# FindoraNetwork/ark-bulletproofs

Hardware: AMD Instinct MI355X
Metric: r1cs_constraints_proved_per_sec (+ r1cs_batch_verifies_per_sec under "verify") (higher is better)
Workload: dtype u32x9 (256-bit modular integers, radix 2^29)

## Files before the change

### ark_bulletproofs_amd/_lib.py

```python
import ctypes as C
import os

import numpy as np

_HERE = os.path.dirname(os.path.abspath(__file__))
LIB_PATH = os.environ.get("ARKBP_LIB_PATH") or os.path.join(_HERE, "libarkbp_hip.so")
_lib = None

BP_OK, BP_E_ARG, BP_E_HIP, BP_E_NO_DEVICE, BP_E_VERIFICATION, BP_E_GENS_LENGTH, BP_E_FORMAT, BP_E_MISSING = 0, -1, -2, -3, -4, -5, -6, -7

EXPORTS = [
    "bp_last_error", "bp_device_count", "bp_ctx_create", "bp_ctx_destroy", "bp_ctx_sync",
    "bp_dev_alloc", "bp_dev_free", "bp_dev_upload", "bp_dev_download", "bp_points_import", "bp_points_export",
    "bp_msm", "bp_msm_gens", "bp_msm_dev", "bp_msm_window_count", "bp_msm_dev_windows", "bp_ipa_create", "bp_ipa_begin", "bp_ipa_round_LR", "bp_ipa_round_fold", "bp_ipa_finish", "bp_ipa_export", "bp_ipa_verify", "bp_gens_derive", "bp_gens_upload", "bp_gens_download", "bp_pedersen_gens",
    "bp_host_derive_generators", "bp_transcript_new", "bp_transcript_free", "bp_transcript_append_message", "bp_transcript_challenge_bytes",
    "bp_transcript_append_point", "bp_transcript_challenge_scalar", "bp_host_sha3_512", "bp_host_points_sum", "bp_debug_rng_draws", "bp_debug_append_points_x8", "bp_debug_challenge_x8", "bp_r1cs_prove_scenario", "bp_stmt_prover_create", "bp_stmt_free", "bp_stmt_info", "bp_stmt_prove", "bp_stmt_precompute", "bp_stmt_precompute_batch", "bp_gens_share", "bp_r1cs_verification_gh", "bp_r1cs_verify_scenario", "bp_r1cs_batch_verify_scenarios", "bp_ctx_set_profiling", "bp_ctx_kernel_time", "bp_ctx_reset_profiling",
    "bp_debug_decompress", "bp_debug_field_op", "bp_debug_point_op", "bp_debug_glv_decompose", "bp_ctx_set_tuning", "bp_ctx_set_window_shard", "bp_pedersen_commit_batch", "bp_stmt_prover_create_dev",
    "bp_prover_new", "bp_verifier_new", "bp_verifier_new_like", "bp_cs_free", "bp_cs_transcript", "bp_cs_metrics", "bp_prover_commit", "bp_verifier_commit",
    "bp_cs_multiply", "bp_cs_allocate", "bp_cs_allocate_multiplier", "bp_cs_constrain", "bp_cs_allocate_multipliers", "bp_cs_constrain_many",
    "bp_cs_specify_randomized_constraints", "bp_cs_challenge_scalar", "bp_prover_set_rng", "bp_prover_precompute", "bp_prover_precompute_batch", "bp_prover_prove", "bp_prover_prove_batch", "bp_prover_commit_batch", "bp_ctx_prove_batch_stats",
    "bp_ctx_set_shard_allgather", "bp_gens_fold_tables", "bp_gens_msm_tables", "bp_debug_exp_iter", "bp_debug_inner_product", "bp_verifier_verify", "bp_r1cs_batch_verify", "bp_stmt_as_prover", "bp_transcript_export_state", "bp_transcript_import_state", "bp_transcript_clone",
    "bp_gens_tables_check", "bp_debug_tables_ptr", "bp_rccl_unique_id", "bp_ctx_rccl_init", "bp_ctx_rccl_shutdown", "bp_ctx_collective_stats", "bp_debug_rccl_allgather",
    "bp_debug_vfe_schedule_replay", "bp_debug_vfe_schedule_replay_2phase", "bp_debug_vfe_challenges", "bp_ctx_vfe_stats", "bp_debug_verify_challenges", "bp_debug_ctx_create_hostonly", "bp_ctx_msm_stats", "bp_ctx_direct_stats", "bp_gens_direct_tables", "bp_ctx_fold_stats", "bp_gens_fold_tables_slice",
]


class ArkbpError(RuntimeError):
    def __init__(self, code, where):
        self.code = code
        msg = lib().bp_last_error().decode(errors="replace") if _lib is not None else ""
        super().__init__("%s failed with code %d: %s" % (where, code, msg))


def lib():
    global _lib
    if _lib is None:
        if not os.path.exists(LIB_PATH):
            raise ImportError(
# ... 25 lines not shown
```

### ark_bulletproofs_amd/csrc/arkbp.hip

```cpp
#include <hip/hip_runtime.h>
#include <sys/prctl.h>
#include <time.h>
#include <rccl/rccl.h>
#include <dlfcn.h>
#include <mutex>
#include <cmath>
#include <cstdio>
#include <cstring>
#include <algorithm>
#include <array>
#include <functional>
#include <map>
#include <memory>
#include <set>
#include <string>
#include <unordered_map>
#include <vector>
#include "../../include/arkbp.h"
#include <atomic>
#include <chrono>
#include "host_proto.hpp"
#include "r1cs.cuh"
#include "pedersen.cuh"
#include "small.cuh"
// ... 153 lines not shown
    bool have_gf = false, have_rho = false;
    F4 gf_halves[2];
    const F4* rho_pw = nullptr;
    const u32* d_rho_pow = nullptr;
    bool lr_done = false;
    bool allow_freeze = false, frozen = false;
    size_t n0 = 0;
    u32 *d_cG = nullptr, *d_cH = nullptr;
    u32 gens_first = 0, gens_stride = 0;
    const u32 *d_G_in = nullptr, *d_H_in = nullptr;
    bool have_qw = false;
    F4 qw;
    int msm_mode = -1;
    bool deferred = false;
    F4 def_tG, def_tH;
    size_t min_len = 0;
    bool direct = false;
    bool fold_pending = false;
    F4 pend_u, pend_ui;
    u32 *d_a_alt = nullptr, *d_b_alt = nullptr;
    F4 geo_k0;
    bool have_k0 = false;
};

struct bp_ctx {
    int curve = 0, device = 0;
    bool host_only = false;
    hipStream_t stream = nullptr;
    bool profiling = false;
    size_t tune_fold_batch_min = 65536;
// ... 49 lines not shown
    void* gather_user = nullptr;
    ncclComm_t nccl = nullptr;
    DevBuf coll_send, coll_recv;
    void* h_coll = nullptr;
    size_t h_coll_cap = 0;
    uint64_t coll_count = 0;
    double coll_seconds = 0;
    size_t tune_cyclic_min = (size_t)1 << 14;
    size_t tune_msm_fixed_min = (size_t)1 << 20;
    size_t tune_host_threads = 0;
    hipEvent_t sync_ev_aux = nullptr;
    unsigned tune_wait_sleep = 0;
    bool msm_latency_first = false;
    size_t tune_msm_chunk_cap = 0;
    size_t tune_fold_quad_max = 0;
    size_t tune_msm_glv_min = 256;
    DevBuf cyc_a, cyc_b, cyc_Gf, cyc_Hf;
    DevBuf fb_G, fb_H, fb_pc;
    size_t fb_cap = 0;
    DevBuf ftab_G, ftab_H;
    size_t ftab_n = 0;
    u32 ftab_first = 0, ftab_stride = 1;
    int ftab_w = 0, ftab_nwin = 0;
    DevBuf dt_tab, dt_part, dt_a2, dt_b2, dt_ticket;
    size_t dt_cap = 0;
    size_t tune_direct_max = 8192;
    u32* h_dt = nullptr;
    u32 dt_pending_parts = 1;
    uint64_t dt_runs = 0;
    size_t tune_prove_batch = 0;
// ... 989 lines not shown
    if constexpr (C::HAS_GLV) {
        Naf2 g, h;
        if (glv_pair<C>(tG, tH, g, h)) {
            if (quad) hipLaunchKernelGGL((k_ipa_fold_glv<C, true>), dim3(grid), dim3(256), 0, st, d_G, d_H, (u32)n, g, h, which, ff.jac);
            else hipLaunchKernelGGL((k_ipa_fold_glv<C, false>), dim3(grid), dim3(256), 0, st, d_G, d_H, (u32)n, g, h, which, ff.jac);
            done = true;
        }
    }
    if (!done) {
        Naf a = naf_of<S>(tG), b = naf_of<S>(tH);
        if (quad) hipLaunchKernelGGL((k_ipa_fold_uniform<C, true>), dim3(grid), dim3(256), 0, st, d_G, d_H, (u32)n, a, b, which, ff.jac);
        else hipLaunchKernelGGL((k_ipa_fold_uniform<C, false>), dim3(grid), dim3(256), 0, st, d_G, d_H, (u32)n, a, b, which, ff.jac);
    }
    }
    fold_finish_launch<C>(ctx, ff, d_G, d_H, n, which, lanes);
    return BP_OK;
}

static void ftab_recode(const uint64_t* mag, int nl, bool negate, int w, int nwin, unsigned short* e, unsigned long long& negmask) {
    uint64_t k[5] = {0, 0, 0, 0, 0};
    for (int i = 0; i < nl; i++) k[i] = mag[i];
    const uint64_t full = (uint64_t)1 << w, half = full >> 1;
    negmask = 0;
    for (int j = 0; j < nwin; j++) {
        uint64_t d = k[0] & (full - 1);
        for (int i = 0; i < 4; i++) k[i] = (k[i] >> w) | (k[i + 1] << (64 - w));
        k[4] >>= w;
        bool neg = false;
        if (d > half) { d = full - d; neg = true; for (int i = 0; i < 5; i++) if (++k[i]) break; }
        e[j] = (unsigned short)d;
        if (d && (neg != negate)) negmask |= 1ull << j;
// ... 297 lines not shown
            s.lr_done = true;
            return BP_OK;
        }
        BaseSegs sg; memset(&sg, 0, sizeof sg);
        sg.nseg = 3; sg.start[0] = 0; sg.start[1] = (u32)n0; sg.start[2] = (u32)(2 * n0); sg.start[3] = (u32)(2 * n0 + 1);
        sg.ptr[0] = s.d_G; sg.ptr[1] = s.d_H; sg.ptr[2] = s.d_Q;
        J4 Lj, Rj;
        BPCHK(msm_run<C>(ctx, sg, sL, 2 * n0 + 1, 0, Lj, 0, -1, s.msm_mode));
        BPCHK(msm_run<C>(ctx, sg, sR, 2 * n0 + 1, 0, Rj, 0, -1, s.msm_mode));
        A4 La = G::to_aff(Lj), Ra = G::to_aff(Rj);
        memcpy(Lw, La.x.v, 32); memcpy(Lw + 4, La.y.v, 32);
        memcpy(Rw, Ra.x.v, 32); memcpy(Rw + 4, Ra.y.v, 32);
        s.lr_done = true;
        return BP_OK;
    }
    if (s.deferred) {
        const size_t n1 = s.n;
        {
            ScopedK tk(ctx, BP_K_IPA_SCALARS);
            hipLaunchKernelGGL(k_ipa_scalars_deferred<C>, dim3(gb), dim3(256), 0, st, s.d_a, s.d_b, (u32)n, sL, sR, ctx->ipa_part.as<u32>(), s.pending ? (s.h_geo ? 2 : 1) : 0,
                               words_of<S>(s.gamma_G), words_of<S>(s.gamma_H), s.d_rho_pow, words_of<S>(s.def_tG), words_of<S>(s.def_tH));
            hipLaunchKernelGGL(k_ipa_ip_finish<C>, dim3(1), dim3(256), 0, st, ctx->ipa_part.as<u32>(), gb, sL + 4 * n * 8, sR + 4 * n * 8, words_of<S>(s.qw), s.have_qw ? 1 : 0);
        }
        J4 Lj, Rj; bool dl = false, dr = false;
        if (s.msm_mode == 2) {
            BaseSegs sg; memset(&sg, 0, sizeof sg);
            sg.nseg = 5;
            for (int k = 0; k <= 4; k++) sg.start[k] = (u32)(k * n);
            sg.start[5] = (u32)(4 * n + 1);
            const size_t f0 = s.gens_first, sd = s.gens_stride;
            const bool rows = s.have_qw && ctx->fb_cap;
            ScalSegs ss; memset(&ss, 0, sizeof ss);
            ss.nseg = 2; ss.ptr[0] = sL; ss.start[0] = 0; ss.start[1] = (u32)(4 * n); ss.ptr[1] = sL + (4 * n + 1) * 8; ss.start[2] = (u32)(4 * n + 1);
            if (rows) {
                FbRun rl[5] = {{0, f0 + (n1 + n) * sd, n, sd}, {0, f0 + n * sd, n, sd}, {1, f0 + n1 * sd, n, sd}, {1, f0, n, sd}, {2, 0, 1}};
                BPCHK(msm_fixed_run<C>(ctx, rl, 5, ss, 4 * n + 1, 0, Lj, dl, 2));
// ... 5 lines not shown
            if (rows) {
                ss.ptr[0] = sR; ss.ptr[1] = sR + (4 * n + 1) * 8;
                FbRun rr[5] = {{0, f0 + n1 * sd, n, sd}, {0, f0, n, sd}, {1, f0 + (n1 + n) * sd, n, sd}, {1, f0 + n * sd, n, sd}, {2, 0, 1}};
                BPCHK(msm_fixed_run<C>(ctx, rr, 5, ss, 4 * n + 1, 0, Rj, dr, 2));
            }
            if (!dr) {
                sg.ptr[0] = s.d_G_in + n1 * 16; sg.ptr[1] = s.d_G_in; sg.ptr[2] = s.d_H_in + (n1 + n) * 16; sg.ptr[3] = s.d_H_in + n * 16; sg.ptr[4] = s.d_Q;
                BPCHK(msm_run<C>(ctx, sg, sR, 4 * n + 1, 0, Rj, 0, -1, 2));
            }
            A4 La = G::to_aff(Lj), Ra = G::to_aff(Rj);
            memcpy(Lw, La.x.v, 32); memcpy(Lw + 4, La.y.v, 32);
            memcpy(Rw, Ra.x.v, 32); memcpy(Rw + 4, Ra.y.v, 32);
            s.lr_done = true;
            return BP_OK;
        }
        const size_t gofs = (size_t)(s.d_G_in - ctx->d_G.as<u32>()) / 16, hofs = (size_t)(s.d_H_in - ctx->d_H.as<u32>()) / 16;
        if (s.have_qw && s.msm_mode == -1) {
            ScalSegs ss; memset(&ss, 0, sizeof ss);
            ss.nseg = 2; ss.ptr[0] = sL; ss.start[0] = 0; ss.start[1] = (u32)(4 * n); ss.ptr[1] = sL + (4 * n + 1) * 8; ss.start[2] = (u32)(4 * n + 1);
            FbRun rl[5] = {{0, gofs + n1 + n, n}, {0, gofs + n, n}, {1, hofs + n1, n}, {1, hofs, n}, {2, 0, 1}};
            BPCHK(msm_fixed_run<C>(ctx, rl, 5, ss, 4 * n + 1, 0, Lj, dl));
            if (dl) {
                ss.ptr[0] = sR; ss.ptr[1] = sR + (4 * n + 1) * 8;
                FbRun rr[5] = {{0, gofs + n1, n}, {0, gofs, n}, {1, hofs + n1 + n, n}, {1, hofs + n, n}, {2, 0, 1}};
                BPCHK(msm_fixed_run<C>(ctx, rr, 5, ss, 4 * n + 1, 0, Rj, dr));
            }
        }
        if (!(dl && dr)) {
            BaseSegs sg; memset(&sg, 0, sizeof sg);
            sg.nseg = 5;
            for (int k = 0; k <= 4; k++) sg.start[k] = (u32)(k * n);
            sg.start[5] = (u32)(4 * n + 1);
            sg.ptr[0] = s.d_G_in + (n1 + n) * 16; sg.ptr[1] = s.d_G_in + n * 16; sg.ptr[2] = s.d_H_in + n1 * 16; sg.ptr[3] = s.d_H_in; sg.ptr[4] = s.d_Q;
            BPCHK(msm_run<C>(ctx, sg, sL, 4 * n + 1, 0, Lj, 0, -1, s.msm_mode));
            sg.ptr[0] = s.d_G_in + n1 * 16; sg.ptr[1] = s.d_G_in; sg.ptr[2] = s.d_H_in + (n1 + n) * 16; sg.ptr[3] = s.d_H_in + n * 16;
            BPCHK(msm_run<C>(ctx, sg, sR, 4 * n + 1, 0, Rj, 0, -1, s.msm_mode));
        }
        A4 La = G::to_aff(Lj), Ra = G::to_aff(Rj);
        memcpy(Lw, La.x.v, 32); memcpy(Lw + 4, La.y.v, 32);
        memcpy(Rw, Ra.x.v, 32); memcpy(Rw + 4, Ra.y.v, 32);
        s.lr_done = true;
        return BP_OK;
    }
    {
        ScopedK tk(ctx, BP_K_IPA_SCALARS);
        hipLaunchKernelGGL(k_ipa_scalars<C>, dim3(gb), dim3(256), 0, st, s.d_a, s.d_b, s.d_Gf, s.d_Hf, s.first ? 1 : 0, (u32)n, sL, sR, ctx->ipa_part.as<u32>(),
                           s.pending ? (s.h_geo ? 2 : 1) : 0, words_of<S>(s.gamma_G), words_of<S>(s.gamma_H), s.d_rho_pow);
        hipLaunchKernelGGL(k_ipa_ip_finish<C>, dim3(1), dim3(256), 0, st, ctx->ipa_part.as<u32>(), gb, sL + 2 * n * 8, sR + 2 * n * 8, words_of<S>(s.qw), s.have_qw ? 1 : 0);
    }
    if (s.d_G_in && s.have_qw && s.msm_mode == -1) {
// ... 133 lines not shown
                BPCHK(launch_tab_fold2<C>(ctx, s, d_G, d_H, n, t2G, t2H, done2));
                if (done2) ctx->folds_tab2++;
                if (!done2) {
                    bool done1 = false;
                    BPCHK(launch_tab_fold<C>(ctx, s, d_G, d_H, 2 * n, s.def_tG, s.def_tH, done1));
                    if (!done1) {
                        if (s.d_G_in != d_G) {
                        HIPCHK(hipMemcpyAsync(d_G, s.d_G_in, 4 * n * 64, hipMemcpyDeviceToDevice, st));
                        HIPCHK(hipMemcpyAsync(d_H, s.d_H_in, 4 * n * 64, hipMemcpyDeviceToDevice, st));
                        }
                        BPCHK(launch_uniform_fold<C>(ctx, d_G, d_H, 2 * n, s.def_tG, s.def_tH, 3));
                    }
                    BPCHK(launch_uniform_fold<C>(ctx, d_G, d_H, n, t2G, t2H, 3));
                }
                s.deferred = false;
            } else
            BPCHK(launch_uniform_fold<C>(ctx, d_G, d_H, n, S::sqr(ui), s.h_geo ? S::mul(S::sqr(u), s.rho_pw[k]) : S::sqr(u), 3));
            s.gamma_G = S::mul(s.gamma_G, u);
            s.gamma_H = s.h_geo ? S::mul(S::mul(s.gamma_H, ui), s.rho_pw[32 + k]) : S::mul(s.gamma_H, ui);
            s.pending = true;
        }
    }
    HIPCHK(hipGetLastError());
    s.first = false;
    if (!s.deferred) s.d_G_in = s.d_H_in = nullptr;
    s.round++;
    s.n = n;
    s.lr_done = false;
    if (s.allow_freeze && n >= 2 && n <= ctx->tune_ipa_freeze_len) {
        BPCHK(ctx->ipa_cG.ensure(n * 32)); BPCHK(ctx->ipa_cH.ensure(n * 32));
        s.d_cG = ctx->ipa_cG.as<u32>(); s.d_cH = ctx->ipa_cH.as<u32>();
        hipLaunchKernelGGL(k_ipa_freeze_init<C>, dim3((u32)((n + 255) / 256)), dim3(256), 0, st, s.d_cG, s.d_cH, (u32)n, s.pending ? (s.h_geo ? 2 : 1) : 0,
// ... 209 lines not shown
    ctx->ipa_step_active = false;
    if (n == 0 || (n & (n - 1))) { g_err = "ipa_begin: n must be a power of two (reference asserts, src/inner_product_proof.rs:66)"; return BP_E_ARG; }
    BPCHK(ipa_upload_host<C>(ctx, Q, Gf, Hf, Gv, Hv, a, b, n));
    BPCHK(ipa_begin_dev<C>(ctx, ctx->ipa_step, ctx->ipa_Q.as<u32>(), ctx->ipa_Gf.as<u32>(), ctx->ipa_Hf.as<u32>(), ctx->ipa_G.as<u32>(), ctx->ipa_H.as<u32>(),
                           ctx->ipa_a.as<u32>(), ctx->ipa_b.as<u32>(), n, nullptr, nullptr, nullptr));
    ctx->ipa_step_active = true;
    return BP_OK;
}
template <class C>
static int ipa_export_host(bp_ctx* ctx, uint64_t* a, uint64_t* b, uint64_t* G_xy, uint64_t* H_xy, uint64_t gG[4], uint64_t gH[4], size_t* n_cur) {
    typedef typename C::Fr Fr;
    IpaState& s = ctx->ipa_step;
    if (s.lr_done) { g_err = "ipa_export: between round_LR and round_fold"; return BP_E_ARG; }
    hipStream_t st = ctx->stream;
    const size_t n = s.n;
    const u32 gb = (u32)((n + 255) / 256);
    BPCHK(ctx->io_out.ensure(n * 64 * 2 + n * 32 * 2));
    u32* o = ctx->io_out.as<u32>();
    hipLaunchKernelGGL(k_points_dev_to_ark<C>, dim3(gb), dim3(256), 0, st, s.d_G, o, (u32)n);
    hipLaunchKernelGGL(k_points_dev_to_ark<C>, dim3(gb), dim3(256), 0, st, s.d_H, o + n * 16, (u32)n);
    hipLaunchKernelGGL(k_scalars_export<Fr>, dim3(gb), dim3(256), 0, st, s.d_a, o + n * 32, (u32)n);
    hipLaunchKernelGGL(k_scalars_export<Fr>, dim3(gb), dim3(256), 0, st, s.d_b, o + n * 40, (u32)n);
    HIPCHK(hipGetLastError());
    HIPCHK(hipMemcpyAsync(G_xy, o, n * 64, hipMemcpyDeviceToHost, st));
    HIPCHK(hipMemcpyAsync(H_xy, o + n * 16, n * 64, hipMemcpyDeviceToHost, st));
    HIPCHK(hipMemcpyAsync(a, o + n * 32, n * 32, hipMemcpyDeviceToHost, st));
    HIPCHK(hipMemcpyAsync(b, o + n * 40, n * 32, hipMemcpyDeviceToHost, st));
    HIPCHK(ctx_stream_wait(ctx));
    memcpy(gG, s.gamma_G.v, 32); memcpy(gH, s.gamma_H.v, 32);
    *n_cur = n;
// ... 582 lines not shown
    c->gather_cb = cb; c->gather_user = user;
    return BP_OK;
}
int bp_ctx_set_tuning(bp_ctx* c, int knob, uint64_t value) {
    if (!c) return BP_E_ARG;
    switch (knob) {
        case BP_TUNE_CYCLIC_MIN: c->tune_cyclic_min = (size_t)value; return BP_OK;
        case BP_TUNE_MSM_FIXED_MIN: c->tune_msm_fixed_min = (size_t)value; return BP_OK;
        case BP_TUNE_HOST_THREADS: if (value > 256) return BP_E_ARG; c->tune_host_threads = (size_t)value; c->pool.reset(); return BP_OK;
        case BP_TUNE_FOLD_BATCH_MIN: c->tune_fold_batch_min = (size_t)value; return BP_OK;
        case BP_TUNE_MSM_BIN_MIN: c->tune_msm_bin_min = (size_t)value; return BP_OK;
        case BP_TUNE_IPA_FREEZE_LEN: c->tune_ipa_freeze_len = (size_t)value; return BP_OK;
        case BP_TUNE_MSM_WSUM_MIN: c->tune_msm_wsum_min = (size_t)value; return BP_OK;
        case BP_TUNE_MSM_GLV_MIN: c->tune_msm_glv_min = (size_t)value; return BP_OK;
        case BP_TUNE_FOLD_QUAD_MAX: c->tune_fold_quad_max = (size_t)value; return BP_OK;
        case BP_TUNE_WAIT_SLEEP: if (value > 1000) return BP_E_ARG; c->tune_wait_sleep = value == 1 ? 30u : (unsigned)value; return BP_OK;
        case BP_TUNE_MSM_CHUNK_CAP: if (value && (value < 8 || value > 64)) return BP_E_ARG; c->tune_msm_chunk_cap = (size_t)value; return BP_OK;
        case BP_TUNE_VFY_DEVICE: c->tune_vfy_device = value >= 2 ? 2 : (int)value; return BP_OK;
        case BP_TUNE_PROVE_BATCH: if (value > 65535) return BP_E_ARG; c->tune_prove_batch = (size_t)value; return BP_OK;
        case BP_TUNE_DIRECT_MAX: if (value > ((uint64_t)1 << 16)) return BP_E_ARG; c->tune_direct_max = (size_t)value; return BP_OK;
    }
    return BP_E_ARG;
}
int bp_ctx_sync(bp_ctx* c) {
    if (!c) return BP_E_ARG;
    HIPCHK(ctx_stream_wait(c));
    return BP_OK;
}

int bp_dev_alloc(bp_ctx* c, size_t bytes, void** dptr) {
// ... 650 lines not shown
    HIPCHK(ctx_stream_wait(c));
    return BP_OK;
}
int bp_debug_verify_challenges(int curve, size_t count, const int* scenarios, const uint64_t* params, const uint8_t* proofs, const size_t* proof_lens,
                               const uint64_t* commit_xy, const size_t* ms, const uint64_t* publics, const size_t* npubs, int use_x8, uint64_t* out, size_t* nchal) {
    if (!count || count > 8 || !scenarios || !params || !proofs || !proof_lens || !commit_xy || !ms || !publics || !npubs || !out || !nchal) return BP_E_ARG;
    return curve == 0 ? dbg_verify_challenges<Secq>(count, scenarios, params, proofs, proof_lens, commit_xy, ms, publics, npubs, use_x8, out, nchal)
                      : dbg_verify_challenges<Zorro>(count, scenarios, params, proofs, proof_lens, commit_xy, ms, publics, npubs, use_x8, out, nchal);
}
int bp_ctx_fold_stats(bp_ctx* c, uint64_t* deferred_first_folds, uint64_t* second_folds_from_tables) {
    if (!c) return BP_E_ARG;
    if (deferred_first_folds) *deferred_first_folds = c->folds_deferred;
    if (second_folds_from_tables) *second_folds_from_tables = c->folds_tab2;
    return BP_OK;
}
int bp_ctx_direct_stats(bp_ctx* c, uint64_t* direct_msms, size_t* bases_per_vector) {
    if (!c) return BP_E_ARG;
    if (direct_msms) *direct_msms = c->dt_runs;
    if (bases_per_vector) *bases_per_vector = c->dt_cap;
    return BP_OK;
}
int bp_ctx_msm_stats(bp_ctx* c, uint64_t* fixed_base_runs, uint64_t* fixed_base_runs_sharded) {
    if (!c) return BP_E_ARG;
    if (fixed_base_runs) *fixed_base_runs = c->fb_runs;
    if (fixed_base_runs_sharded) *fixed_base_runs_sharded = c->fb_runs_sharded;
    return BP_OK;
}
int bp_ctx_vfe_stats(bp_ctx* c, uint64_t* device_batches, uint64_t* host_fallbacks) {
    if (!c) return BP_E_ARG;
    if (device_batches) *device_batches = c->vfe_batches;
// ... 69 lines not shown
```

### ark_bulletproofs_amd/csrc/ipa.cuh

```cuda
#pragma once
#include "msm.cuh"

namespace arkbp {

template <class F> __global__ void k_scalars_import(const u32* __restrict__ in, u32* __restrict__ out, u32 n) {
    const u32 i = blockIdx.x * blockDim.x + threadIdx.x;
    if (i >= n) return;
    u32 w[8];
    load_words8(w, in + (size_t)i * 8);
    store_fe_dev<F>(out + (size_t)i * 8, fe_load_ark<F>(w));
}
template <class F> __global__ void k_scalars_export(const u32* __restrict__ in, u32* __restrict__ out, u32 n) {
    const u32 i = blockIdx.x * blockDim.x + threadIdx.x;
    if (i >= n) return;
    u32 w[8];
    fe_store_ark<F>(w, load_fe_dev<F>(in + (size_t)i * 8));
    store_words8(out + (size_t)i * 8, w);
}

static constexpr int IMPORT_MAX = 5;
struct ImportList {
    u32* dst[IMPORT_MAX];
    u32 cnt[IMPORT_MAX];
    int nseg;
// ... 379 lines not shown
                    const u32 nz = h ? (c | d) : (a | b), ng = h ? d : b;
                    if ((nz >> bit) & 1) {
                        Aff T;
#pragma unroll
                        for (int l = 0; l < 9; l++) { T.x.l[l] = h ? Q1.x.l[l] : P1.x.l[l]; T.y.l[l] = ((ng >> bit) & 1) ? N1.y.l[l] : P1.y.l[l]; }
                        acc = ladder_madd<C>(acc, T);
                    }
                }
            }
        }
    }
    acc = QUAD ? qjac_madd<C>(acc, P2, ql) : jac_madd<C>(acc, P2);
    if (!QUAD || ql == 0) fold_emit<C>(V, i, t, acc, jac_ws);
}

struct FtabDigits {
    unsigned short e1[44], e2[44];
    unsigned long long neg1, neg2;
    u32 nwin;
};
template <class C> __global__ void __launch_bounds__(256)
k_ftab_window(const u32* __restrict__ gens, u32* __restrict__ state, u32* __restrict__ tmp, u32 n, u32 E, int first) {
    const u32 i = blockIdx.x * blockDim.x + threadIdx.x;
    if (i >= n) return;
    Jac B;
    if (first) { const Aff p = load_aff_dev(gens + (size_t)i * 16); B = jac_madd<C>(jac_inf<C>(), p); }
    else B = load_jac_ws(state + (size_t)i * 24);
    Jac acc = B;
    store_jac_ws<C>(tmp + (size_t)i * 24, acc);
#pragma unroll 1
// ... 165 lines not shown
```

### ark_bulletproofs_amd/engine.py

```python
import ctypes as C

import numpy as np

from . import _lib
from ._lib import ArkbpError, check, lib, ptr, u64arr

SECQ256K1, ZORRO = 0, 1


class DeviceBuffer:

    def __init__(self, eng, nbytes):
        self.eng, self.nbytes = eng, nbytes
        p = C.c_void_p()
        check(lib().bp_dev_alloc(eng.ctx, C.c_size_t(nbytes), C.byref(p)), "bp_dev_alloc")
        self.ptr = p

    def upload(self, arr):
        arr = np.ascontiguousarray(arr)
        assert arr.nbytes <= self.nbytes
        check(lib().bp_dev_upload(self.eng.ctx, self.ptr, ptr(arr), C.c_size_t(arr.nbytes)), "bp_dev_upload")
        return self

    def download(self, dtype=np.uint64, nbytes=None):
# ... 909 lines not shown
    return nbytes.value


Engine.gens_direct_tables = _gens_direct_tables


def _fold_stats(self):
    a, b = C.c_uint64(0), C.c_uint64(0)
    check(lib().bp_ctx_fold_stats(self.ctx, C.byref(a), C.byref(b)), "bp_ctx_fold_stats")
    return a.value, b.value


Engine.fold_stats = _fold_stats


def _prover_handle(p):
    if isinstance(p, Statement):
        return C.c_void_p(lib().bp_stmt_as_prover(p.h))
    return p.h


def _prove_batch(self, provers, rng_bytes=None, timing=None, return_rc=False):
    n = len(provers)
    if n == 0:
        return (0, []) if return_rc else []
    hs = (C.c_void_p * n)(*[_prover_handle(p) for p in provers])
    rb = None
    if rng_bytes is not None:
        if len(rng_bytes) != n or any(len(r) != 32 for r in rng_bytes):
            raise ValueError("prove_batch: one 32-byte rng string per instance")
# ... 50 lines not shown
```

### include/arkbp.h

```cpp
#ifndef ARKBP_H
#define ARKBP_H
#include <stddef.h>
#include <stdint.h>
#ifdef __cplusplus
extern "C" {
#endif

#define BP_CURVE_SECQ256K1 0
#define BP_CURVE_ZORRO 1

#define BP_OK 0
#define BP_E_ARG (-1)
#define BP_E_HIP (-2)
#define BP_E_NO_DEVICE (-3)
#define BP_E_VERIFICATION (-4)
#define BP_E_GENS_LENGTH (-5)
#define BP_E_FORMAT (-6)
#define BP_E_MISSING (-7)

typedef struct bp_ctx bp_ctx;

const char* bp_last_error(void);
int bp_device_count(void);
int bp_ctx_create(int curve, int device, bp_ctx** out);
// ... 158 lines not shown

#define BP_TUNE_FOLD_BATCH_MIN 0
#define BP_TUNE_MSM_BIN_MIN 1
#define BP_TUNE_IPA_FREEZE_LEN 2
#define BP_TUNE_MSM_WSUM_MIN 3
#define BP_TUNE_CYCLIC_MIN 4
#define BP_TUNE_MSM_FIXED_MIN 5
#define BP_TUNE_HOST_THREADS 6
#define BP_TUNE_FOLD_QUAD_MAX 8
#define BP_TUNE_MSM_GLV_MIN 7
#define BP_TUNE_WAIT_SLEEP 10
#define BP_TUNE_MSM_CHUNK_CAP 9
#define BP_TUNE_VFY_DEVICE 11
#define BP_TUNE_DIRECT_MAX 12
#define BP_TUNE_PROVE_BATCH 13
int bp_ctx_set_tuning(bp_ctx* ctx, int knob, uint64_t value);

int bp_r1cs_verification_gh(bp_ctx* ctx, size_t n, size_t n1, const uint64_t* wL, const uint64_t* wR, const uint64_t* wO, const uint64_t y[4],
                            const uint64_t x[4], const uint64_t u[4], const uint64_t a[4], const uint64_t b[4], const uint64_t* ipa_challenges, size_t k,
                            uint64_t* g_out, uint64_t* h_out);

int bp_debug_field_op(bp_ctx* ctx, int field, int op, const uint64_t* a, const uint64_t* b, uint64_t* out, size_t n);
int bp_debug_exp_iter(bp_ctx* ctx, const uint64_t x[4], size_t n, uint64_t* out);
int bp_debug_inner_product(bp_ctx* ctx, const uint64_t* a, const uint64_t* b, size_t n, uint64_t out[4]);
int bp_debug_decompress(bp_ctx* ctx, const uint8_t* compressed33, size_t n, uint64_t* out_xy, uint32_t* out_ok);
int bp_debug_glv_decompose(int curve, const uint64_t t[4], uint32_t masks[20], uint64_t lambda_out[4]);
int bp_debug_vfe_schedule_replay(const uint8_t state203[203], int absorb_commitments, uint64_t m, uint32_t k, uint64_t n, const uint8_t* items, uint8_t* seeds_out,
                                 uint32_t* nblocks_out);
int bp_debug_vfe_schedule_replay_2phase(const uint8_t state203[203], int absorb_commitments, uint64_t m, uint32_t k, uint64_t n, const char* const* labels, size_t nlabels,
                                        const uint8_t* items, uint8_t* seeds_out, uint32_t* nblocks_out);
int bp_debug_vfe_challenges(bp_ctx* ctx, size_t count, const uint8_t* proofs, size_t proof_len, const uint64_t* commit_xy, size_t m, const uint8_t* states203,
                            int shared_state, int absorb_commitments, uint8_t* seeds_out, uint64_t* chal_out, uint32_t* status_out);
int bp_ctx_vfe_stats(bp_ctx* ctx, uint64_t* device_batches, uint64_t* host_fallbacks);
int bp_ctx_msm_stats(bp_ctx* ctx, uint64_t* fixed_base_runs, uint64_t* fixed_base_runs_sharded);
int bp_ctx_direct_stats(bp_ctx* ctx, uint64_t* direct_msms, size_t* bases_per_vector);
int bp_ctx_fold_stats(bp_ctx* ctx, uint64_t* deferred_first_folds, uint64_t* second_folds_from_tables);
int bp_debug_ctx_create_hostonly(int curve, size_t gens_capacity, bp_ctx** out);
int bp_debug_verify_challenges(int curve, size_t count, const int* scenarios, const uint64_t* params, const uint8_t* proofs, const size_t* proof_lens,
                               const uint64_t* commit_xy, const size_t* ms, const uint64_t* publics, const size_t* npubs, int use_x8, uint64_t* out,
                               size_t* nchal);
int bp_debug_point_op(bp_ctx* ctx, int op, const uint64_t* p_xy, const uint64_t* q_xy, const uint64_t* k, uint64_t* out_xy, size_t n);

#ifdef __cplusplus
}
#endif
#endif
```

### shim/src/ffi.rs

```rust
#![allow(non_camel_case_types, non_snake_case, clippy::too_many_arguments, clippy::missing_safety_doc)]
use core::ffi::{c_char, c_int, c_void};

#[repr(C)] pub struct BpCtx { _private: [u8; 0] }
#[repr(C)] pub struct BpCs { _private: [u8; 0] }
#[repr(C)] pub struct BpStmt { _private: [u8; 0] }
#[repr(C)] #[derive(Clone, Copy, Debug, Default, PartialEq, Eq)] pub struct BpVar { pub kind: u32, pub index: u32 }

pub const BP_CURVE_SECQ256K1: c_int = 0;
pub const BP_CURVE_ZORRO: c_int = 1;
pub const BP_OK: c_int = 0;
pub const BP_E_ARG: c_int = -1;
pub const BP_E_HIP: c_int = -2;
pub const BP_E_NO_DEVICE: c_int = -3;
pub const BP_E_VERIFICATION: c_int = -4;
pub const BP_E_GENS_LENGTH: c_int = -5;
pub const BP_E_FORMAT: c_int = -6;
pub const BP_E_MISSING: c_int = -7;
pub const BP_VAR_COMMITTED: c_int = 0;
pub const BP_VAR_MULT_LEFT: c_int = 1;
pub const BP_VAR_MULT_RIGHT: c_int = 2;
pub const BP_VAR_MULT_OUT: c_int = 3;
pub const BP_VAR_ONE: c_int = 4;
pub const BP_K_MSM_ACCUM: c_int = 0;
pub const BP_K_MSM_TOTAL: c_int = 1;
// ... 13 lines not shown
pub const BP_K_COUNT: c_int = 15;
pub const BP_TUNE_FOLD_BATCH_MIN: c_int = 0;
pub const BP_TUNE_MSM_BIN_MIN: c_int = 1;
pub const BP_TUNE_IPA_FREEZE_LEN: c_int = 2;
pub const BP_TUNE_MSM_WSUM_MIN: c_int = 3;
pub const BP_TUNE_CYCLIC_MIN: c_int = 4;
pub const BP_TUNE_MSM_FIXED_MIN: c_int = 5;
pub const BP_TUNE_HOST_THREADS: c_int = 6;
pub const BP_TUNE_FOLD_QUAD_MAX: c_int = 8;
pub const BP_TUNE_MSM_GLV_MIN: c_int = 7;
pub const BP_TUNE_WAIT_SLEEP: c_int = 10;
pub const BP_TUNE_MSM_CHUNK_CAP: c_int = 9;
pub const BP_TUNE_VFY_DEVICE: c_int = 11;
pub const BP_TUNE_DIRECT_MAX: c_int = 12;
pub const BP_TUNE_PROVE_BATCH: c_int = 13;

pub type BpPointReduceCb = unsafe extern "C" fn(user: *mut c_void, xy: *mut u64) -> c_int;
pub type BpAllgatherCb = unsafe extern "C" fn(user: *mut c_void, send: *const c_void, bytes: usize, recv: *mut c_void) -> c_int;
pub type BpChallengeCb = unsafe extern "C" fn(user: *mut c_void, l_xy: *const u64, r_xy: *const u64, u_out: *mut u64) -> c_int;
pub type BpRandomizeCb = unsafe extern "C" fn(user: *mut c_void, cs: *mut BpCs) -> c_int;

#[link(name = "arkbp_hip")]
extern "C" {
    pub fn bp_last_error() -> *const c_char;
    pub fn bp_device_count() -> c_int;
    pub fn bp_ctx_create(curve: c_int, device: c_int, out: *mut *mut BpCtx) -> c_int;
    pub fn bp_ctx_destroy(ctx: *mut BpCtx);
    pub fn bp_ctx_sync(ctx: *mut BpCtx) -> c_int;
    pub fn bp_dev_alloc(ctx: *mut BpCtx, bytes: usize, dptr: *mut *mut c_void) -> c_int;
    pub fn bp_dev_free(ctx: *mut BpCtx, dptr: *mut c_void) -> c_int;
// ... 88 lines not shown
    pub fn bp_ctx_reset_profiling(ctx: *mut BpCtx) -> c_int;
    pub fn bp_ctx_set_tuning(ctx: *mut BpCtx, knob: c_int, value: u64) -> c_int;
    pub fn bp_r1cs_verification_gh(ctx: *mut BpCtx, n: usize, n1: usize, wL: *const u64, wR: *const u64, wO: *const u64, y: *const u64, x: *const u64, u: *const u64, a: *const u64, b: *const u64, ipa_challenges: *const u64, k: usize, g_out: *mut u64, h_out: *mut u64) -> c_int;
    pub fn bp_debug_field_op(ctx: *mut BpCtx, field: c_int, op: c_int, a: *const u64, b: *const u64, out: *mut u64, n: usize) -> c_int;
    pub fn bp_debug_exp_iter(ctx: *mut BpCtx, x: *const u64, n: usize, out: *mut u64) -> c_int;
    pub fn bp_debug_inner_product(ctx: *mut BpCtx, a: *const u64, b: *const u64, n: usize, out: *mut u64) -> c_int;
    pub fn bp_debug_decompress(ctx: *mut BpCtx, compressed33: *const u8, n: usize, out_xy: *mut u64, out_ok: *mut u32) -> c_int;
    pub fn bp_debug_glv_decompose(curve: c_int, t: *const u64, masks: *mut u32, lambda_out: *mut u64) -> c_int;
    pub fn bp_debug_vfe_schedule_replay(state203: *const u8, absorb_commitments: c_int, m: u64, k: u32, n: u64, items: *const u8, seeds_out: *mut u8, nblocks_out: *mut u32) -> c_int;
    pub fn bp_debug_vfe_schedule_replay_2phase(state203: *const u8, absorb_commitments: c_int, m: u64, k: u32, n: u64, labels: *const *const c_char, nlabels: usize, items: *const u8, seeds_out: *mut u8, nblocks_out: *mut u32) -> c_int;
    pub fn bp_debug_vfe_challenges(ctx: *mut BpCtx, count: usize, proofs: *const u8, proof_len: usize, commit_xy: *const u64, m: usize, states203: *const u8, shared_state: c_int, absorb_commitments: c_int, seeds_out: *mut u8, chal_out: *mut u64, status_out: *mut u32) -> c_int;
    pub fn bp_ctx_vfe_stats(ctx: *mut BpCtx, device_batches: *mut u64, host_fallbacks: *mut u64) -> c_int;
    pub fn bp_ctx_msm_stats(ctx: *mut BpCtx, fixed_base_runs: *mut u64, fixed_base_runs_sharded: *mut u64) -> c_int;
    pub fn bp_ctx_direct_stats(ctx: *mut BpCtx, direct_msms: *mut u64, bases_per_vector: *mut usize) -> c_int;
    pub fn bp_ctx_fold_stats(ctx: *mut BpCtx, deferred_first_folds: *mut u64, second_folds_from_tables: *mut u64) -> c_int;
    pub fn bp_debug_ctx_create_hostonly(curve: c_int, gens_capacity: usize, out: *mut *mut BpCtx) -> c_int;
    pub fn bp_debug_verify_challenges(curve: c_int, count: usize, scenarios: *const c_int, params: *const u64, proofs: *const u8, proof_lens: *const usize, commit_xy: *const u64, ms: *const usize, publics: *const u64, npubs: *const usize, use_x8: c_int, out: *mut u64, nchal: *mut usize) -> c_int;
    pub fn bp_debug_point_op(ctx: *mut BpCtx, op: c_int, p_xy: *const u64, q_xy: *const u64, k: *const u64, out_xy: *mut u64, n: usize) -> c_int;
}
```

Baseline: 15.24 million.

## Pair consecutive IPA generator folds into one multi-scalar ladder pass

Defers the generator fold of one IPA round and merges it with the next round's fold. A new kernel computes each output point as a 4-term combination (three scalar products via a shared double-and-add ladder over combined NAF/GLV digits, plus one unscaled point). The next round's L/R MSMs read the unfolded generators with the deferred scalars folded into the scalar vectors. This halves the number of fold ladder passes over G/H at the cost of more adds per pass, extra LDS staging and more deferral bookkeeping, and it is enabled by default for eligible sizes.

```diff
diff --git a/ark_bulletproofs_amd/_lib.py b/ark_bulletproofs_amd/_lib.py
--- a/ark_bulletproofs_amd/_lib.py
+++ b/ark_bulletproofs_amd/_lib.py
@@ -21,7 +21,7 @@
     "bp_cs_specify_randomized_constraints", "bp_cs_challenge_scalar", "bp_prover_set_rng", "bp_prover_precompute", "bp_prover_precompute_batch", "bp_prover_prove", "bp_prover_prove_batch", "bp_prover_commit_batch", "bp_ctx_prove_batch_stats",
     "bp_ctx_set_shard_allgather", "bp_gens_fold_tables", "bp_gens_msm_tables", "bp_debug_exp_iter", "bp_debug_inner_product", "bp_verifier_verify", "bp_r1cs_batch_verify", "bp_stmt_as_prover", "bp_transcript_export_state", "bp_transcript_import_state", "bp_transcript_clone",
     "bp_gens_tables_check", "bp_debug_tables_ptr", "bp_rccl_unique_id", "bp_ctx_rccl_init", "bp_ctx_rccl_shutdown", "bp_ctx_collective_stats", "bp_debug_rccl_allgather",
-    "bp_debug_vfe_schedule_replay", "bp_debug_vfe_schedule_replay_2phase", "bp_debug_vfe_challenges", "bp_ctx_vfe_stats", "bp_debug_verify_challenges", "bp_debug_ctx_create_hostonly", "bp_ctx_msm_stats", "bp_ctx_direct_stats", "bp_gens_direct_tables", "bp_ctx_fold_stats", "bp_gens_fold_tables_slice",
+    "bp_debug_vfe_schedule_replay", "bp_debug_vfe_schedule_replay_2phase", "bp_debug_vfe_challenges", "bp_ctx_vfe_stats", "bp_debug_verify_challenges", "bp_debug_ctx_create_hostonly", "bp_ctx_msm_stats", "bp_ctx_direct_stats", "bp_gens_direct_tables", "bp_ctx_fold_stats", "bp_gens_fold_tables_slice", "bp_ctx_ladder_stats",
 ]
 
 
diff --git a/ark_bulletproofs_amd/csrc/arkbp.hip b/ark_bulletproofs_amd/csrc/arkbp.hip
--- a/ark_bulletproofs_amd/csrc/arkbp.hip
+++ b/ark_bulletproofs_amd/csrc/arkbp.hip
@@ -191,6 +191,8 @@
     int msm_mode = -1;
     bool deferred = false;
     F4 def_tG, def_tH;
+    bool pair_def = false;
+    F4 pair_tG, pair_tH;
     size_t min_len = 0;
     bool direct = false;
     bool fold_pending = false;
@@ -270,6 +272,8 @@
     bool msm_latency_first = false;
     size_t tune_msm_chunk_cap = 0;
     size_t tune_fold_quad_max = 0;
+    size_t tune_fold_pair_min = 1;
+    uint64_t ladder_paired = 0, ladder_single = 0;
     size_t tune_msm_glv_min = 256;
     DevBuf cyc_a, cyc_b, cyc_Gf, cyc_Hf;
     DevBuf fb_G, fb_H, fb_pc;
@@ -1289,7 +1293,56 @@
     }
     }
     fold_finish_launch<C>(ctx, ff, d_G, d_H, n, which, lanes);
-    return BP_OK;
+    ctx->ladder_single++;
+    return BP_OK;
+}
+template <class C> static int launch_pair_fold(bp_ctx* ctx, u32* d_G, u32* d_H, size_t n, const F4& t1G, const F4& t2G, const F4& t1H, const F4& t2H, bool& done) {
+    typedef host::Fld<typename C::Fr> S;
+    done = false;
+    const F4 mG[3] = {t1G, t2G, S::mul(t1G, t2G)}, mH[3] = {t1H, t2H, S::mul(t1H, t2H)};
+    const u32 lanes = (u32)(2 * n), grid = (lanes + PAIR_BLOCK - 1) / PAIR_BLOCK;
+    FoldFinish ff;
+    if constexpr (C::HAS_GLV) {
+        PairDigits<6, 5> g, h;
+        for (int v = 0; v < 2; v++) {
+            PairDigits<6, 5>& d = v ? h : g;
+            for (int k = 0; k < 3; k++) {
+                u32 p1[5], m1[5], p2[5], m2[5];
+                if (!glv_decompose<C>(v ? mH[k] : mG[k], p1, m1, p2, m2)) return BP_OK;
+                for (int w = 0; w < 5; w++) { d.nz[2 * k][w] = p1[w] | m1[w]; d.ng[2 * k][w] = m1[w]; d.nz[2 * k + 1][w] = p2[w] | m2[w]; d.ng[2 * k + 1][w] = m2[w]; }
+            }
+        }
+        BPCHK(fold_finish_plan(ctx, lanes, ff));
+        ScopedK tk(ctx, BP_K_FOLD_LADDER);
+        static const bool wpe2 = getenv("ARKBP_PAIR_WPE2") != nullptr;
+        if (wpe2) hipLaunchKernelGGL((k_ipa_fold_pair<C, true, 2>), dim3(grid), dim3(PAIR_BLOCK), 0, ctx->stream, d_G, d_H, (u32)n, g, h, 3, ff.jac);
+        else
+        hipLaunchKernelGGL((k_ipa_fold_pair<C, true>), dim3(grid), dim3(PAIR_BLOCK), 0, ctx->stream, d_G, d_H, (u32)n, g, h, 3, ff.jac);
+    } else {
+        PairDigits<3, 9> g, h;
+        for (int v = 0; v < 2; v++) {
+            PairDigits<3, 9>& d = v ? h : g;
+            for (int k = 0; k < 3; k++) {
+                const Naf a = naf_of<S>(v ? mH[k] : mG[k]);
+                for (int w = 0; w < 9; w++) { d.nz[k][w] = a.plus[w] | a.minus[w]; d.ng[k][w] = a.minus[w]; }
+            }
+        }
+        BPCHK(fold_finish_plan(ctx, lanes, ff));
+        ScopedK tk(ctx, BP_K_FOLD_LADDER);
+        hipLaunchKernelGGL((k_ipa_fold_pair<C, false>), dim3(grid), dim3(PAIR_BLOCK), 0, ctx->stream, d_G, d_H, (u32)n, g, h, 3, ff.jac);
+    }
+    fold_finish_launch<C>(ctx, ff, d_G, d_H, n, 3, lanes);
+    ctx->ladder_paired++;
+    done = true;
+    return BP_OK;
+}
+static bool fold_can_pair(const bp_ctx* ctx, const IpaState& s, size_t n) {
+    static const bool off = getenv("ARKBP_FOLD_NOPAIR") != nullptr;
+    if (off || !ctx->tune_fold_pair_min || s.msm_mode != -1 || ctx->shard_world != 1 || n < 2 || n < ctx->tune_fold_pair_min) return false;
+    const size_t q = ctx->tune_fold_quad_max;
+    if ((2 * n >= 64 && 2 * n <= q) || (n >= 64 && n <= q)) return false;
+    if (s.allow_freeze && ctx->tune_ipa_freeze_len >= 2 && n / 2 < ctx->tune_ipa_freeze_len) return false;
+    return true;
 }
 
 static void ftab_recode(const uint64_t* mag, int nl, bool negate, int w, int nwin, unsigned short* e, unsigned long long& negmask) {
@@ -1617,12 +1670,14 @@
         s.lr_done = true;
         return BP_OK;
     }
-    if (s.deferred) {
+    if (s.deferred || s.pair_def) {
         const size_t n1 = s.n;
+        const u32 *Gu = s.pair_def ? s.d_G : s.d_G_in, *Hu = s.pair_def ? s.d_H : s.d_H_in;
+        const F4 &dtG = s.pair_def ? s.pair_tG : s.def_tG, &dtH = s.pair_def ? s.pair_tH : s.def_tH;
         {
             ScopedK tk(ctx, BP_K_IPA_SCALARS);
             hipLaunchKernelGGL(k_ipa_scalars_deferred<C>, dim3(gb), dim3(256), 0, st, s.d_a, s.d_b, (u32)n, sL, sR, ctx->ipa_part.as<u32>(), s.pending ? (s.h_geo ? 2 : 1) : 0,
-                               words_of<S>(s.gamma_G), words_of<S>(s.gamma_H), s.d_rho_pow, words_of<S>(s.def_tG), words_of<S>(s.def_tH));
+                               words_of<S>(s.gamma_G), words_of<S>(s.gamma_H), s.d_rho_pow, words_of<S>(dtG), words_of<S>(dtH));
             hipLaunchKernelGGL(k_ipa_ip_finish<C>, dim3(1), dim3(256), 0, st, ctx->ipa_part.as<u32>(), gb, sL + 4 * n * 8, sR + 4 * n * 8, words_of<S>(s.qw), s.have_qw ? 1 : 0);
         }
         J4 Lj, Rj; bool dl = false, dr = false;
@@ -1658,8 +1713,8 @@
             s.lr_done = true;
             return BP_OK;
         }
-        const size_t gofs = (size_t)(s.d_G_in - ctx->d_G.as<u32>()) / 16, hofs = (size_t)(s.d_H_in - ctx->d_H.as<u32>()) / 16;
-        if (s.have_qw && s.msm_mode == -1) {
+        if (!s.pair_def && s.have_qw && s.msm_mode == -1) {
+            const size_t gofs = (size_t)(s.d_G_in - ctx->d_G.as<u32>()) / 16, hofs = (size_t)(s.d_H_in - ctx->d_H.as<u32>()) / 16;
             ScalSegs ss; memset(&ss, 0, sizeof ss);
             ss.nseg = 2; ss.ptr[0] = sL; ss.start[0] = 0; ss.start[1] = (u32)(4 * n); ss.ptr[1] = sL + (4 * n + 1) * 8; ss.start[2] = (u32)(4 * n + 1);
             FbRun rl[5] = {{0, gofs + n1 + n, n}, {0, gofs + n, n}, {1, hofs + n1, n}, {1, hofs, n}, {2, 0, 1}};
@@ -1675,9 +1730,9 @@
             sg.nseg = 5;
             for (int k = 0; k <= 4; k++) sg.start[k] = (u32)(k * n);
             sg.start[5] = (u32)(4 * n + 1);
-            sg.ptr[0] = s.d_G_in + (n1 + n) * 16; sg.ptr[1] = s.d_G_in + n * 16; sg.ptr[2] = s.d_H_in + n1 * 16; sg.ptr[3] = s.d_H_in; sg.ptr[4] = s.d_Q;
+            sg.ptr[0] = Gu + (n1 + n) * 16; sg.ptr[1] = Gu + n * 16; sg.ptr[2] = Hu + n1 * 16; sg.ptr[3] = Hu; sg.ptr[4] = s.d_Q;
             BPCHK(msm_run<C>(ctx, sg, sL, 4 * n + 1, 0, Lj, 0, -1, s.msm_mode));
-            sg.ptr[0] = s.d_G_in + n1 * 16; sg.ptr[1] = s.d_G_in; sg.ptr[2] = s.d_H_in + (n1 + n) * 16; sg.ptr[3] = s.d_H_in + n * 16;
+            sg.ptr[0] = Gu + n1 * 16; sg.ptr[1] = Gu; sg.ptr[2] = Hu + (n1 + n) * 16; sg.ptr[3] = Hu + n * 16;
             BPCHK(msm_run<C>(ctx, sg, sR, 4 * n + 1, 0, Rj, 0, -1, s.msm_mode));
         }
         A4 La = G::to_aff(Lj), Ra = G::to_aff(Rj);
@@ -1841,8 +1896,18 @@
                     BPCHK(launch_uniform_fold<C>(ctx, d_G, d_H, n, t2G, t2H, 3));
                 }
                 s.deferred = false;
+            } else if (s.pair_def) {
+                bool done2 = false;
+                BPCHK(launch_pair_fold<C>(ctx, d_G, d_H, n, s.pair_tG, t2G, s.pair_tH, t2H, done2));
+                if (!done2) {
+                    BPCHK(launch_uniform_fold<C>(ctx, d_G, d_H, 2 * n, s.pair_tG, s.pair_tH, 3));
+                    BPCHK(launch_uniform_fold<C>(ctx, d_G, d_H, n, t2G, t2H, 3));
+                }
+                s.pair_def = false;
+            } else if (fold_can_pair(ctx, s, n)) {
+                s.pair_def = true; s.pair_tG = t2G; s.pair_tH = t2H;
             } else
-            BPCHK(launch_uniform_fold<C>(ctx, d_G, d_H, n, S::sqr(ui), s.h_geo ? S::mul(S::sqr(u), s.rho_pw[k]) : S::sqr(u), 3));
+            BPCHK(launch_uniform_fold<C>(ctx, d_G, d_H, n, t2G, t2H, 3));
             s.gamma_G = S::mul(s.gamma_G, u);
             s.gamma_H = s.h_geo ? S::mul(S::mul(s.gamma_H, ui), s.rho_pw[32 + k]) : S::mul(s.gamma_H, ui);
             s.pending = true;
@@ -2082,6 +2147,10 @@
     if (s.lr_done) { g_err = "ipa_export: between round_LR and round_fold"; return BP_E_ARG; }
     hipStream_t st = ctx->stream;
     const size_t n = s.n;
+    if (s.pair_def) {
+        BPCHK(launch_uniform_fold<C>(ctx, s.d_G, s.d_H, n, s.pair_tG, s.pair_tH, 3));
+        s.pair_def = false;
+    }
     const u32 gb = (u32)((n + 255) / 256);
     BPCHK(ctx->io_out.ensure(n * 64 * 2 + n * 32 * 2));
     u32* o = ctx->io_out.as<u32>();
@@ -2694,6 +2763,7 @@
         case BP_TUNE_MSM_WSUM_MIN: c->tune_msm_wsum_min = (size_t)value; return BP_OK;
         case BP_TUNE_MSM_GLV_MIN: c->tune_msm_glv_min = (size_t)value; return BP_OK;
         case BP_TUNE_FOLD_QUAD_MAX: c->tune_fold_quad_max = (size_t)value; return BP_OK;
+        case BP_TUNE_FOLD_PAIR_MIN: c->tune_fold_pair_min = (size_t)value; return BP_OK;
         case BP_TUNE_WAIT_SLEEP: if (value > 1000) return BP_E_ARG; c->tune_wait_sleep = value == 1 ? 30u : (unsigned)value; return BP_OK;
         case BP_TUNE_MSM_CHUNK_CAP: if (value && (value < 8 || value > 64)) return BP_E_ARG; c->tune_msm_chunk_cap = (size_t)value; return BP_OK;
         case BP_TUNE_VFY_DEVICE: c->tune_vfy_device = value >= 2 ? 2 : (int)value; return BP_OK;
@@ -3374,6 +3444,12 @@
     if (second_folds_from_tables) *second_folds_from_tables = c->folds_tab2;
     return BP_OK;
 }
+int bp_ctx_ladder_stats(bp_ctx* c, uint64_t* paired_passes, uint64_t* single_passes) {
+    if (!c) return BP_E_ARG;
+    if (paired_passes) *paired_passes = c->ladder_paired;
+    if (single_passes) *single_passes = c->ladder_single;
+    return BP_OK;
+}
 int bp_ctx_direct_stats(bp_ctx* c, uint64_t* direct_msms, size_t* bases_per_vector) {
     if (!c) return BP_E_ARG;
     if (direct_msms) *direct_msms = c->dt_runs;
diff --git a/ark_bulletproofs_amd/csrc/ipa.cuh b/ark_bulletproofs_amd/csrc/ipa.cuh
--- a/ark_bulletproofs_amd/csrc/ipa.cuh
+++ b/ark_bulletproofs_amd/csrc/ipa.cuh
@@ -417,6 +417,73 @@
     if (!QUAD || ql == 0) fold_emit<C>(V, i, t, acc, jac_ws);
 }
 
+template <int NS, int NW> struct PairDigits {
+    u32 nz[NS][NW], ng[NS][NW];
+};
+static constexpr int PAIR_BLOCK = 128;
+__device__ __forceinline__ Fe pair_lds_fe(const uint4* __restrict__ my, u32 slot) {
+    const uint4 a = my[(slot * 2) * PAIR_BLOCK], b = my[(slot * 2 + 1) * PAIR_BLOCK];
+    const u32 w[8] = {a.x, a.y, a.z, a.w, b.x, b.y, b.z, b.w};
+    return fe_unpack(w);
+}
+__device__ __forceinline__ void pair_lds_put(uint4* __restrict__ my, u32 slot, const u32 w[8]) {
+    my[(slot * 2) * PAIR_BLOCK] = make_uint4(w[0], w[1], w[2], w[3]);
+    my[(slot * 2 + 1) * PAIR_BLOCK] = make_uint4(w[4], w[5], w[6], w[7]);
+}
+template <class C, bool GLV, int WPE = (GLV ? 3 : 2)> __global__ void __launch_bounds__(PAIR_BLOCK) __attribute__((amdgpu_waves_per_eu(WPE)))
+k_ipa_fold_pair(u32* __restrict__ G, u32* __restrict__ H, u32 n, PairDigits<(GLV ? 6 : 3), (GLV ? 5 : 9)> dG, PairDigits<(GLV ? 6 : 3), (GLV ? 5 : 9)> dH,
+                int which , u32* __restrict__ jac_ws) {
+    typedef typename C::Fq F;
+    constexpr int NS = GLV ? 6 : 3, NW = GLV ? 5 : 9, SL = GLV ? 3 : 2;
+    __shared__ uint4 sh[3 * SL * 2 * PAIR_BLOCK];
+    const u32 t = blockIdx.x * PAIR_BLOCK + threadIdx.x;
+    if (t >= (which == 3 ? 2 * n : n)) return;
+    const bool isH = which == 2 || (which == 3 && t >= n);
+    const u32 i = (which == 3 && isH) ? t - n : t;
+    u32* V = isH ? H : G;
+    uint4* my = sh + threadIdx.x;
+#pragma unroll
+    for (int k = 0; k < 3; k++) {
+        const u32* src = V + ((size_t)(k == 0 ? 1 : k == 1 ? 2 : 0) * n + i) * 16;
+        u32 w[16];
+        load_words8(w, src);
+        load_words8(w + 8, src + 8);
+        pair_lds_put(my, k * SL, w);
+        pair_lds_put(my, k * SL + 1, w + 8);
+        if constexpr (GLV) {
+            u32 bx[8];
+            fe_pack(bx, fe_canon<F>(fe_mul<F>(fe_unpack(w), fe_const<F, C::BETA29>())));
+            pair_lds_put(my, k * SL + 2, bx);
+        }
+    }
+    Jac acc = jac_inf<C>();
+#pragma unroll 1
+    for (int wd = NW - 1; wd >= 0; wd--) {
+        u32 nz[NS], ng[NS];
+#pragma unroll
+        for (int s = 0; s < NS; s++) { nz[s] = isH ? dH.nz[s][wd] : dG.nz[s][wd]; ng[s] = isH ? dH.ng[s][wd] : dG.ng[s][wd]; }
+#pragma unroll 1
+        for (int bit = (wd == NW - 1 ? (GLV ? 1 : 0) : 31); bit >= 0; bit--) {
+            acc = jac_dbl<C>(acc);
+            u32 m = 0, g = 0;
+#pragma unroll
+            for (int s = 0; s < NS; s++) { m |= ((nz[s] >> bit) & 1u) << s; g |= ((ng[s] >> bit) & 1u) << s; }
+#pragma unroll 1
+            while (m) {
+                const u32 s = (u32)__ffs((int)m) - 1u;
+                m &= m - 1u;
+                const u32 k = GLV ? s >> 1 : s;
+                Aff T;
+                T.x = pair_lds_fe(my, k * SL + ((GLV && (s & 1u)) ? 2u : 0u));
+                T.y = pair_lds_fe(my, k * SL + 1u);
+                acc = ladder_madd<C>(acc, aff_cneg_lazy<C>(T, ((g >> s) & 1u) != 0));
+            }
+        }
+    }
+    acc = jac_madd<C>(acc, load_aff_dev(V + ((size_t)3 * n + i) * 16));
+    fold_emit<C>(V, i, t, acc, jac_ws);
+}
+
 struct FtabDigits {
     unsigned short e1[44], e2[44];
     unsigned long long neg1, neg2;
diff --git a/ark_bulletproofs_amd/engine.py b/ark_bulletproofs_amd/engine.py
--- a/ark_bulletproofs_amd/engine.py
+++ b/ark_bulletproofs_amd/engine.py
@@ -947,6 +947,15 @@
 Engine.fold_stats = _fold_stats
 
 
+def _ladder_stats(self):
+    a, b = C.c_uint64(0), C.c_uint64(0)
+    check(lib().bp_ctx_ladder_stats(self.ctx, C.byref(a), C.byref(b)), "bp_ctx_ladder_stats")
+    return a.value, b.value
+
+
+Engine.ladder_stats = _ladder_stats
+
+
 def _prover_handle(p):
     if isinstance(p, Statement):
         return C.c_void_p(lib().bp_stmt_as_prover(p.h))
diff --git a/include/arkbp.h b/include/arkbp.h
--- a/include/arkbp.h
+++ b/include/arkbp.h
@@ -196,6 +196,7 @@
 #define BP_TUNE_VFY_DEVICE 11
 #define BP_TUNE_DIRECT_MAX 12
 #define BP_TUNE_PROVE_BATCH 13
+#define BP_TUNE_FOLD_PAIR_MIN 14
 int bp_ctx_set_tuning(bp_ctx* ctx, int knob, uint64_t value);
 
 int bp_r1cs_verification_gh(bp_ctx* ctx, size_t n, size_t n1, const uint64_t* wL, const uint64_t* wR, const uint64_t* wO, const uint64_t y[4],
@@ -217,6 +218,7 @@
 int bp_ctx_msm_stats(bp_ctx* ctx, uint64_t* fixed_base_runs, uint64_t* fixed_base_runs_sharded);
 int bp_ctx_direct_stats(bp_ctx* ctx, uint64_t* direct_msms, size_t* bases_per_vector);
 int bp_ctx_fold_stats(bp_ctx* ctx, uint64_t* deferred_first_folds, uint64_t* second_folds_from_tables);
+int bp_ctx_ladder_stats(bp_ctx* ctx, uint64_t* paired_passes, uint64_t* single_passes);
 int bp_debug_ctx_create_hostonly(int curve, size_t gens_capacity, bp_ctx** out);
 int bp_debug_verify_challenges(int curve, size_t count, const int* scenarios, const uint64_t* params, const uint8_t* proofs, const size_t* proof_lens,
                                const uint64_t* commit_xy, const size_t* ms, const uint64_t* publics, const size_t* npubs, int use_x8, uint64_t* out,
diff --git a/shim/src/ffi.rs b/shim/src/ffi.rs
--- a/shim/src/ffi.rs
+++ b/shim/src/ffi.rs
@@ -51,6 +51,7 @@
 pub const BP_TUNE_VFY_DEVICE: c_int = 11;
 pub const BP_TUNE_DIRECT_MAX: c_int = 12;
 pub const BP_TUNE_PROVE_BATCH: c_int = 13;
+pub const BP_TUNE_FOLD_PAIR_MIN: c_int = 14;
 
 pub type BpPointReduceCb = unsafe extern "C" fn(user: *mut c_void, xy: *mut u64) -> c_int;
 pub type BpAllgatherCb = unsafe extern "C" fn(user: *mut c_void, send: *const c_void, bytes: usize, recv: *mut c_void) -> c_int;
@@ -169,6 +170,7 @@
     pub fn bp_ctx_msm_stats(ctx: *mut BpCtx, fixed_base_runs: *mut u64, fixed_base_runs_sharded: *mut u64) -> c_int;
     pub fn bp_ctx_direct_stats(ctx: *mut BpCtx, direct_msms: *mut u64, bases_per_vector: *mut usize) -> c_int;
     pub fn bp_ctx_fold_stats(ctx: *mut BpCtx, deferred_first_folds: *mut u64, second_folds_from_tables: *mut u64) -> c_int;
+    pub fn bp_ctx_ladder_stats(ctx: *mut BpCtx, paired_passes: *mut u64, single_passes: *mut u64) -> c_int;
     pub fn bp_debug_ctx_create_hostonly(curve: c_int, gens_capacity: usize, out: *mut *mut BpCtx) -> c_int;
     pub fn bp_debug_verify_challenges(curve: c_int, count: usize, scenarios: *const c_int, params: *const u64, proofs: *const u8, proof_lens: *const usize, commit_xy: *const u64, ms: *const usize, publics: *const u64, npubs: *const usize, use_x8: c_int, out: *mut u64, nchal: *mut usize) -> c_int;
     pub fn bp_debug_point_op(ctx: *mut BpCtx, op: c_int, p_xy: *const u64, q_xy: *const u64, k: *const u64, out_xy: *mut u64, n: usize) -> c_int;
```

After: 17.25 million, median of 4. +13.2%, better.
